# niclasborlin/dbat

Hardware: NVIDIA B200
Metric: lm_iterations_per_s (higher is better)
Workload: dtype f64

## Files before the change

dbat_b200/csrc/api.cu:

```cuda
#include <algorithm>
#include <chrono>
#include <cmath>
#include <cstdio>
#include <cstring>
#include <map>
#include <string>
#include <iterator>
#include <vector>
#include <condition_variable>
#include <functional>
#include <memory>
#include <mutex>
#include <thread>
#include <dlfcn.h>

#include "../../include/dbat_gpu.h"
#include "kernels.cuh"
#include "launch.h"
#include "tilechol.h"

int64_t g_dbat_launches = 0;
static std::string g_create_err;

#define CK(call)                                                                                   \
// ... 431 lines not shown
            for (int sl = 0; sl < DBAT_NSLOT; ++sl) {
                const int c = h->h_io_colx[(size_t)i * DBAT_NSLOT + sl];
                if (c >= 0 && lastUser[c] != i) { users[c]++; lastUser[c] = i; }
            }
        h->h_glob_x.clear();
        h->h_colLocalImg.assign(std::max(1, nC), -1);
        for (int c = 0; c < nC; ++c) {
            if (users[c] >= 2 || (users[c] == 1 && !general)) h->h_glob_x.push_back(c);
            else if (users[c] == 1) { h->h_colLocalImg[c] = lastUser[c]; h->h_nEO[lastUser[c]]++; }
        }
        h->h_nIOest = (int)h->h_glob_x.size();
        if ((rc = setup_reduced(h, 1, 0))) return fail_create(h, rc, h->err);
    }
    const std::vector<int>& imgRank = h->tc.sym.imgRank;
    AL(P.chunkG, (size_t)std::max(1, P.nChunks) * DBAT_GSZ);
    {
        const size_t nCp = (size_t)std::max(1, nC);
        h->nEvalRed = (size_t)nImg * DBAT_GSZ + DBAT_GSZ + 2 * nCp + 8;
        AL(h->d_evalRed, h->nEvalRed);
        P.imgG = h->d_evalRed;
        P.shG = P.imgG + (size_t)nImg * DBAT_GSZ;
        h->d_camDiag = P.shG + DBAT_GSZ;
        h->d_camG = h->d_camDiag + nCp;
        h->d_prr = h->d_camG + nCp;
        cudaMemset(h->d_camDiag, 0, sizeof(double) * (2 * nCp + 8));
    }
    AL(P.pt, (size_t)std::max(1, nOP) * DBAT_PT_STRIDE);
    cudaMemset(P.pt, 0, sizeof(double) * (size_t)std::max(1, nOP) * DBAT_PT_STRIDE);
    {
        bool ok = !general && nK <= 3 && nP <= 2 && getenv("DBAT_EVAL_GENERIC") == nullptr;
        for (int sl = 0; sl < DBAT_NSLOT; ++sl) if (h->h_sh_col[sl] >= 0 && !((0x0CEFu >> sl) & 1)) ok = false;
        P.evalCompact = ok ? 1 : 0;
    }
    AL(P.W, (size_t)std::max(1, nObs) * DBAT_W_STRIDE);
    if (P.ioGeneral) AL(P.Wfull, (size_t)std::max(1, nObs) * DBAT_WF_STRIDE);
    {
        std::vector<int> pt_pm(nObs);
        for (int o = 0; o < nObs; ++o) pt_pm[o] = h->h_pt_cm[h->h_pm2cm[o]];
        int* d_pt_pm;
        UP(d_pt_pm, pt_pm);
        P.pt_pm = d_pt_pm;
    }
    {
        std::vector<int> pairs, bigp;
        int begin = 0, cnt = 0;
        auto close = [&](int end) { if (end > begin) { pairs.push_back(begin); pairs.push_back(end); } begin = end; cnt = 0; };
        for (int j = 0; j < nOP; ++j) {
            const int k = h->h_pt_start[j + 1] - h->h_pt_start[j];
            if (k > DBAT_PSB) { close(j); bigp.push_back(j); begin = j + 1; continue; }
            if (cnt + k > DBAT_PSB || j - begin >= DBAT_PSB / 2) close(j);
            cnt += k;
        }
        close(nOP);
        P.nPsb = (int)pairs.size() / 2;
        P.nPsbig = (int)bigp.size();
        if (pairs.empty()) pairs.assign(2, 0);
        if (bigp.empty()) bigp.push_back(0);
        int *d_pairs, *d_bigp;
        UP(d_pairs, pairs); UP(d_bigp, bigp);
        P.psb_pt = d_pairs; P.psbig = d_bigp;
    }
    {
        std::vector<int> cand, big;
        cand.reserve(nOP);
        int maxm = DBAT_GRP_MAXM;
        if (const char* e = getenv("DBAT_GRP_MAXM")) maxm = std::max(1, std::min(DBAT_GRP_MAXM, atoi(e)));
        for (int j = 0; j < nOP; ++j) {
// ... 994 lines not shown
    res->launches = g_dbat_launches - l0;
    CK(cudaMemcpyAsync(res->x, h->d_x, sizeof(double) * nn, cudaMemcpyDeviceToHost, h->st));
    if (res->p) CK(cudaMemcpyAsync(res->p, h->d_p, sizeof(double) * nn, cudaMemcpyDeviceToHost, h->st));
    if (res->r_w || res->r_u) {
        set_params(h, h->d_x); h->params_valid = true;
        if (res->r_w) {
            launch_resid(h->P, h->d_x, h->d_partial, h->d_scal, SC_PRR, h->d_r, 1, h->st);
            CK(cudaMemcpyAsync(res->r_w, h->d_r, sizeof(double) * h->m, cudaMemcpyDeviceToHost, h->st));
            CK(cudaStreamSynchronize(h->st));
        }
        if (res->r_u) {
            launch_resid(h->P, h->d_x, h->d_partial, h->d_scal, SC_PRR, h->d_r, 0, h->st);
            CK(cudaMemcpyAsync(res->r_u, h->d_r, sizeof(double) * h->m, cudaMemcpyDeviceToHost, h->st));
        }
    }
    ph_collect(h);
    CK(cudaStreamSynchronize(h->st));
    return DBAT_OK;
}

__global__ void __launch_bounds__(128) k_cop(DevProblem P, const double* __restrict__ C, int ldc,
                                              const double* __restrict__ dsc, double s02, double* __restrict__ out);


__global__ void k_cov_rows(DevProblem P, double* __restrict__ T, int* __restrict__ Tc) {
    const int j = blockIdx.x * blockDim.x + threadIdx.x;
    if (j >= P.nOP) return;
    const size_t r0 = (size_t)DBAT_NSLOT * j + 6 * (size_t)P.pt_start[j];
    const int o0 = P.pt_start[j], k = P.pt_start[j + 1] - o0;
    const double* rec = P.pt + (size_t)j * DBAT_PT_STRIDE;
    const double* v = P.vinv + (size_t)j * 8;
    const double Vi[6] = {v[0], v[1], v[2], v[3], v[4], v[5]};
    for (int a = 0; a < DBAT_NSLOT + 6 * k; ++a) {
        const double* w; int col;
        if (a < DBAT_NSLOT) { w = rec + DBAT_PT_WSH + 3 * a; col = P.sh_s[a]; }
        else {
            const int o = (a - DBAT_NSLOT) / 6, e = (a - DBAT_NSLOT) % 6;
            w = P.W + (size_t)(o0 + o) * DBAT_W_STRIDE + 3 * e;
            col = P.eo_s[6 * (size_t)P.img_pm[o0 + o] + e];
        }
        double* t = T + 3 * (r0 + a);
        t[0] = Vi[0] * w[0] + Vi[1] * w[1] + Vi[2] * w[2];
        t[1] = Vi[1] * w[0] + Vi[3] * w[1] + Vi[4] * w[2];
        t[2] = Vi[2] * w[0] + Vi[4] * w[1] + Vi[5] * w[2];
        Tc[r0 + a] = col;
    }
}
__global__ void k_cov_U(DevProblem P, const double* __restrict__ C, int ldc, const double* __restrict__ dsc,
                        const double* __restrict__ T, const int* __restrict__ Tc, const int* __restrict__ x2s,
                        double* __restrict__ U) {
    const int rx = blockIdx.x * blockDim.x + threadIdx.x, j = blockIdx.y;
    if (rx >= P.nC) return;
    const int r = x2s[rx];
    const int* opc = P.op_col + 3 * (size_t)j;
    if (opc[0] < 0 && opc[1] < 0 && opc[2] < 0) return;
    const size_t r0 = (size_t)DBAT_NSLOT * j + 6 * (size_t)P.pt_start[j];
    const int rows = DBAT_NSLOT + 6 * (P.pt_start[j + 1] - P.pt_start[j]);
    double u[3] = {0.0, 0.0, 0.0};
    const double dr = dsc[r];
    for (int a = 0; a < rows; ++a) {
        const int ca = Tc[r0 + a];
        if (ca < 0) continue;
        const double c = C[(size_t)ca * ldc + r] * dr * dsc[ca];
        const double* t = T + 3 * (r0 + a);
        u[0] += c * t[0]; u[1] += c * t[1]; u[2] += c * t[2];
    }
    for (int t = 0; t < 3; ++t) if (opc[t] >= 0) U[(size_t)(opc[t] - P.nC) * P.nC + rx] = u[t];
}
__global__ void k_cov_pp(DevProblem P, const double* __restrict__ T, const int* __restrict__ Tc,
                         const double* __restrict__ U, const int* __restrict__ col2pt, double* __restrict__ Cpp) {
    const int m3 = P.n - P.nC;
// ... 250 lines not shown
    if (info != 0) { for (int c = 0; c < P.n; ++c) std_x[c] = NAN; return DBAT_E_NOTSPD; }
    return DBAT_OK;
}

__global__ void __launch_bounds__(128) k_cop(DevProblem P, const double* __restrict__ C, int ldc,
                                              const double* __restrict__ dsc, double s02, double* __restrict__ out) {
    const int lane = threadIdx.x & 31;
    const int j = (blockIdx.x * blockDim.x + threadIdx.x) >> 5;
    if (j >= P.nOP) return;
    const int* opc = P.op_col + 3 * (size_t)j;
    if (opc[0] < 0 && opc[1] < 0 && opc[2] < 0) return;
    const double* rec = P.pt + (size_t)j * DBAT_PT_STRIDE;
    double a00 = rec[0], a01 = rec[1], a02 = rec[2], a11 = rec[3], a12 = rec[4], a22 = rec[5];
    const bool f0 = opc[0] >= 0, f1 = opc[1] >= 0, f2 = opc[2] >= 0;
    if (!f0) a00 = 1.0; if (!f1) a11 = 1.0; if (!f2) a22 = 1.0;
    const double l00 = sqrt(a00), l10 = a01 / l00, l20 = a02 / l00;
    const double l11 = sqrt(a11 - l10 * l10), l21 = (a12 - l20 * l10) / l11;
    const double l22 = sqrt(a22 - l20 * l20 - l21 * l21);
    const double m00 = 1.0 / l00, m11 = 1.0 / l11, m22 = 1.0 / l22;
    const double m10 = -l10 * m00 * m11, m21 = -l21 * m11 * m22, m20 = -(l20 * m00 + l21 * m10) * m22;
    double Vi[6] = {m00 * m00 + m10 * m10 + m20 * m20, m10 * m11 + m20 * m21, m20 * m22,
                    m11 * m11 + m21 * m21, m21 * m22, m22 * m22};
    if (!f0) { Vi[0] = 0; Vi[1] = 0; Vi[2] = 0; }
    if (!f1) { Vi[1] = 0; Vi[3] = 0; Vi[4] = 0; }
    if (!f2) { Vi[2] = 0; Vi[4] = 0; Vi[5] = 0; }
    const int o0 = P.pt_start[j], k = P.pt_start[j + 1] - o0;
    const int nRows = DBAT_NSLOT + 6 * k;
    auto row_col = [&](int a) -> int {
        if (a < DBAT_NSLOT) return P.sh_s[a];
        const int o = (a - DBAT_NSLOT) / 6, e = (a - DBAT_NSLOT) % 6;
        return P.eo_s[6 * (size_t)P.img_pm[o0 + o] + e];
    };
    auto row_T = [&](int a, double T[3]) {
        const double* w = (a < DBAT_NSLOT) ? rec + DBAT_PT_WSH + 3 * a
                                           : P.W + (size_t)(o0 + (a - DBAT_NSLOT) / 6) * DBAT_W_STRIDE + 3 * ((a - DBAT_NSLOT) % 6);
        T[0] = Vi[0] * w[0] + Vi[1] * w[1] + Vi[2] * w[2];
        T[1] = Vi[1] * w[0] + Vi[3] * w[1] + Vi[4] * w[2];
        T[2] = Vi[2] * w[0] + Vi[4] * w[1] + Vi[5] * w[2];
    };
    double acc[6] = {0, 0, 0, 0, 0, 0};
    for (int a = lane; a < nRows; a += 32) {
        const int ca = row_col(a);
        if (ca < 0) continue;
        double Ta[3]; row_T(a, Ta);
        double u[3] = {0, 0, 0};
        for (int b = 0; b < nRows; ++b) {
            const int cb = row_col(b);
            if (cb < 0) continue;
            double Tb[3]; row_T(b, Tb);
            const double c = C[(size_t)cb * ldc + ca] * dsc[ca] * dsc[cb];
            u[0] += c * Tb[0]; u[1] += c * Tb[1]; u[2] += c * Tb[2];
        }
        acc[0] += Ta[0] * u[0]; acc[1] += Ta[0] * u[1]; acc[2] += Ta[0] * u[2];
        acc[3] += Ta[1] * u[1]; acc[4] += Ta[1] * u[2]; acc[5] += Ta[2] * u[2];
    }
#pragma unroll
    for (int q = 0; q < 6; ++q)
#pragma unroll
        for (int o = 16; o > 0; o >>= 1) acc[q] += __shfl_xor_sync(0xffffffffu, acc[q], o);
    if (lane == 0) {
        double* o9 = out + 9 * (size_t)j;
        const double c00 = s02 * (Vi[0] + acc[0]), c01 = s02 * (Vi[1] + acc[1]), c02 = s02 * (Vi[2] + acc[2]);
        const double c11 = s02 * (Vi[3] + acc[3]), c12 = s02 * (Vi[4] + acc[4]), c22 = s02 * (Vi[5] + acc[5]);
        o9[0] = c00; o9[1] = c01; o9[2] = c02; o9[3] = c01; o9[4] = c11; o9[5] = c12; o9[6] = c02; o9[7] = c12; o9[8] = c22;
    }
}

extern "C" int dbat_dense_chol_solve(int64_t n, const double* A, const double* b, double* x, double* Ainv,
// ... 452 lines not shown
```

dbat_b200/csrc/eval.cu:

```cuda
#include "kernels.cuh"
#include "launch.h"

__device__ __forceinline__ double warp_sum(double v) {
#pragma unroll
    for (int o = 16; o > 0; o >>= 1) v += __shfl_xor_sync(0xffffffffu, v, o);
    return v;
}

__device__ __forceinline__ double block_sum(double v, double* sm ) {
    v = warp_sum(v);
    const int w = threadIdx.x >> 5, l = threadIdx.x & 31;
    __syncthreads();
    if (l == 0) sm[w] = v;
    __syncthreads();
    double t = 0.0;
    if (w == 0) {
        t = (l < (int)(blockDim.x >> 5)) ? sm[l] : 0.0;
        t = warp_sum(t);
    }
    return t;
}

__global__ void __launch_bounds__(256) k_scatter3(const double* __restrict__ x, ScatterList a, ScatterList b, ScatterList c) {
    int blk = blockIdx.x;
// ... 333 lines not shown
    double m[3];
#pragma unroll
    for (int t = 0; t < 3; ++t) m[t] = P.op_col[3 * (size_t)j + t] >= 0 ? 1.0 : 0.0;
    double V[6] = {0, 0, 0, 0, 0, 0}, gq[3] = {0, 0, 0};
    double Wsh[DBAT_NSLOT][3];
#pragma unroll
    for (int s = 0; s < DBAT_NSLOT; ++s) { Wsh[s][0] = 0.0; Wsh[s][1] = 0.0; Wsh[s][2] = 0.0; }
    const int o0 = P.pt_start[j], o1 = P.pt_start[j + 1];
    for (int ob = o0; ob < o1; ++ob) {
        const double2 uv = P.uv_pm[ob];
        const double2 is = P.isig_pm[ob];
        const ImgRec g = P.img[P.img_pm[ob]];
        const IORec io = P.io[g.io];
        ObsJac o;
        obs_model<MODEL, true, true>(Q, g, io, P.nK, P.nP, uv.x, uv.y, o);
        double A[2][3];
#pragma unroll
        for (int t = 0; t < 3; ++t) { A[0][t] = o.dOP[0][t] * is.x * m[t]; A[1][t] = o.dOP[1][t] * is.y * m[t]; }
        const double r0 = o.r[0] * is.x, r1 = o.r[1] * is.y;
        V[0] += A[0][0] * A[0][0] + A[1][0] * A[1][0];
        V[1] += A[0][0] * A[0][1] + A[1][0] * A[1][1];
        V[2] += A[0][0] * A[0][2] + A[1][0] * A[1][2];
        V[3] += A[0][1] * A[0][1] + A[1][1] * A[1][1];
        V[4] += A[0][1] * A[0][2] + A[1][1] * A[1][2];
        V[5] += A[0][2] * A[0][2] + A[1][2] * A[1][2];
#pragma unroll
        for (int t = 0; t < 3; ++t) gq[t] += A[0][t] * r0 + A[1][t] * r1;
#pragma unroll
        for (int s = 0; s < DBAT_NSLOT; ++s) {
            const double a0 = o.dIO[s][0] * is.x, a1 = o.dIO[s][1] * is.y;
#pragma unroll
            for (int t = 0; t < 3; ++t) Wsh[s][t] += a0 * A[0][t] + a1 * A[1][t];
        }
        double* Wo = P.W + (size_t)ob * DBAT_W_STRIDE;
#pragma unroll
        for (int c = 0; c < 3; ++c) {
            const double a0 = o.dC[0][c] * is.x, a1 = o.dC[1][c] * is.y;
            const double b0 = o.dA[0][c] * is.x, b1 = o.dA[1][c] * is.y;
#pragma unroll
            for (int t = 0; t < 3; ++t) {
                Wo[c * 3 + t] = a0 * A[0][t] + a1 * A[1][t];
                Wo[(3 + c) * 3 + t] = b0 * A[0][t] + b1 * A[1][t];
            }
        }
    }
    double* rec = P.pt + (size_t)j * DBAT_PT_STRIDE;
#pragma unroll
    for (int k = 0; k < 6; ++k) rec[k] = V[k];
#pragma unroll
    for (int t = 0; t < 3; ++t) rec[6 + t] = gq[t];
    rec[9] = 0.0;
#pragma unroll
    for (int s = 0; s < DBAT_NSLOT; ++s)
#pragma unroll
        for (int t = 0; t < 3; ++t) rec[DBAT_PT_WSH + 3 * s + t] = Wsh[s][t];
}

__global__ void k_prior_apply(DevProblem P, const double* __restrict__ x,
                              double* __restrict__ camDiag, double* __restrict__ camG,
                              const int* __restrict__ col2pt ) {
    const int k = blockIdx.x * blockDim.x + threadIdx.x;
    if (k >= P.nPrior) return;
    const int c = P.prior_col[k];
    const double w = P.prior_isig[k];
    const double r = (x[c] - P.prior_val[k]) * w;
    if (c < P.nC) {
        camDiag[c] += w * w;
        camG[c] += w * r;
    } else {
        const int e = col2pt[c - P.nC];
        const int j = e / 3, t = e % 3;
        double* rec = P.pt + (size_t)j * DBAT_PT_STRIDE;
        const int d = (t == 0) ? 0 : (t == 1 ? 3 : 5);
        rec[d] += w * w;
        rec[6 + t] += w * r;
    }
}
// ... 7 lines not shown
    const int ob0 = P.pt_start[p0], nob = P.pt_start[p1] - ob0;
    if (tid < nob) {
        const int ob = ob0 + tid;
        const int j = P.pt_pm[ob];
        const double2 uv = P.uv_pm[ob];
        const double2 is = P.isig_pm[ob];
        const ImgRec g = P.img[P.img_pm[ob]];
        const IORec io = P.io[g.io];
        const double Q[3] = {P.OPval[3 * (size_t)j], P.OPval[3 * (size_t)j + 1], P.OPval[3 * (size_t)j + 2]};
        ObsJac o;
        obs_model<MODEL, true, true>(Q, g, io, P.nK, P.nP, uv.x, uv.y, o);
        double* row = rows + tid * PS_ROW;
        double A[2][3];
#pragma unroll
        for (int t = 0; t < 3; ++t) {
            const double m = P.op_col[3 * (size_t)j + t] >= 0 ? 1.0 : 0.0;
            A[0][t] = o.dOP[0][t] * is.x * m; A[1][t] = o.dOP[1][t] * is.y * m;
            row[t] = A[0][t]; row[3 + t] = A[1][t];
        }
        row[6] = o.r[0] * is.x; row[7] = o.r[1] * is.y;
#pragma unroll
        for (int s = 0; s < DBAT_NSLOT; ++s) { row[8 + 2 * s] = o.dIO[s][0] * is.x; row[9 + 2 * s] = o.dIO[s][1] * is.y; }
        double w[18];
#pragma unroll
        for (int c = 0; c < 3; ++c) {
            const double a0 = o.dC[0][c] * is.x, a1 = o.dC[1][c] * is.y;
            const double b0 = o.dA[0][c] * is.x, b1 = o.dA[1][c] * is.y;
#pragma unroll
            for (int t = 0; t < 3; ++t) {
                w[c * 3 + t] = a0 * A[0][t] + a1 * A[1][t];
                w[(3 + c) * 3 + t] = b0 * A[0][t] + b1 * A[1][t];
            }
        }
        double2* Wo = reinterpret_cast<double2*>(P.W + (size_t)ob * DBAT_W_STRIDE);
#pragma unroll
        for (int q = 0; q < 9; ++q) Wo[q] = make_double2(w[2 * q], w[2 * q + 1]);
    }
    __syncthreads();
    const int nItems = (p1 - p0) * 16;
    for (int item = tid; item < nItems; item += DBAT_PSB) {
        const int j = p0 + (item >> 4), it = item & 15;
        const int r0 = P.pt_start[j] - ob0, r1 = P.pt_start[j + 1] - ob0;
        double* rec = P.pt + (size_t)j * DBAT_PT_STRIDE;
        if (it < DBAT_NSLOT) {
            double a0 = 0.0, a1 = 0.0, a2 = 0.0;
            for (int r = r0; r < r1; ++r) {
                const double* row = rows + r * PS_ROW;
                const double u0 = row[8 + 2 * it], u1 = row[9 + 2 * it];
                a0 += u0 * row[0] + u1 * row[3]; a1 += u0 * row[1] + u1 * row[4]; a2 += u0 * row[2] + u1 * row[5];
            }
            rec[DBAT_PT_WSH + 3 * it] = a0; rec[DBAT_PT_WSH + 3 * it + 1] = a1; rec[DBAT_PT_WSH + 3 * it + 2] = a2;
        } else if (it == 14) {
            double V[6] = {0, 0, 0, 0, 0, 0};
            for (int r = r0; r < r1; ++r) {
                const double* row = rows + r * PS_ROW;
                V[0] += row[0] * row[0] + row[3] * row[3];
                V[1] += row[0] * row[1] + row[3] * row[4];
                V[2] += row[0] * row[2] + row[3] * row[5];
                V[3] += row[1] * row[1] + row[4] * row[4];
                V[4] += row[1] * row[2] + row[4] * row[5];
                V[5] += row[2] * row[2] + row[5] * row[5];
            }
#pragma unroll
            for (int k = 0; k < 6; ++k) rec[k] = V[k];
        } else {
            double g0 = 0.0, g1 = 0.0, g2 = 0.0;
            for (int r = r0; r < r1; ++r) {
                const double* row = rows + r * PS_ROW;
                g0 += row[0] * row[6] + row[3] * row[7]; g1 += row[1] * row[6] + row[4] * row[7]; g2 += row[2] * row[6] + row[5] * row[7];
            }
            rec[6] = g0; rec[7] = g1; rec[8] = g2; rec[9] = 0.0;
        }
    }
}

#define PSC_ROW 27
__device__ __constant__ unsigned char c_ceSlot[CE_NA] = {0, 1, 2, 3, 5, 6, 7, 10, 11};
#ifndef PSC_MINB
#define PSC_MINB 5
#endif
template <int MODEL>
__global__ void __launch_bounds__(DBAT_PSB, PSC_MINB) k_point_side_obs_c(DevProblem P) {
    __shared__ __align__(16) double rows[DBAT_PSB * PSC_ROW];
    const int tid = threadIdx.x, lane = tid & 31;
    const int p0 = P.psb_pt[2 * blockIdx.x], p1 = P.psb_pt[2 * blockIdx.x + 1];
    const int ob0 = P.pt_start[p0], nob = P.pt_start[p1] - ob0;
    const bool valid = tid < nob;
    ObsJac o;
    double A[2][3];
    double2 is = make_double2(0.0, 0.0);
    double* stage = rows + (tid - lane) * PSC_ROW;
    if (valid) {
        const int ob = ob0 + tid;
        const int j = P.pt_pm[ob];
        const double2 uv = P.uv_pm[ob];
        is = P.isig_pm[ob];
        const ImgRec g = P.img[P.img_pm[ob]];
        const IORec io = P.io[g.io];
        const double Q[3] = {P.OPval[3 * (size_t)j], P.OPval[3 * (size_t)j + 1], P.OPval[3 * (size_t)j + 2]};
        obs_model<MODEL, true, true>(Q, g, io, CE_NK, CE_NP, uv.x, uv.y, o);
#pragma unroll
        for (int t = 0; t < 3; ++t) {
            const double m = P.op_col[3 * (size_t)j + t] >= 0 ? 1.0 : 0.0;
            A[0][t] = o.dOP[0][t] * is.x * m; A[1][t] = o.dOP[1][t] * is.y * m;
        }
        double w[18];
#pragma unroll
        for (int c = 0; c < 3; ++c) {
            const double a0 = o.dC[0][c] * is.x, a1 = o.dC[1][c] * is.y;
            const double b0 = o.dA[0][c] * is.x, b1 = o.dA[1][c] * is.y;
#pragma unroll
            for (int t = 0; t < 3; ++t) {
                w[c * 3 + t] = a0 * A[0][t] + a1 * A[1][t];
                w[(3 + c) * 3 + t] = b0 * A[0][t] + b1 * A[1][t];
            }
        }
        double2* sw = reinterpret_cast<double2*>(stage + lane * DBAT_W_STRIDE);
#pragma unroll
        for (int q = 0; q < 9; ++q) sw[q] = make_double2(w[2 * q], w[2 * q + 1]);
    }
    __syncwarp();
    {
        const int nv = min(32, nob - (tid - lane));
        double2* Wg = reinterpret_cast<double2*>(P.W + (size_t)(ob0 + tid - lane) * DBAT_W_STRIDE);
        const double2* ss = reinterpret_cast<const double2*>(stage);
#pragma unroll
        for (int q = 0; q < 9; ++q) {
            const int piece = q * 32 + lane;
            if (piece < nv * 9) Wg[piece] = ss[piece];
        }
    }
    __syncwarp();
    if (valid) {
        double* row = rows + tid * PSC_ROW;
#pragma unroll
        for (int t = 0; t < 3; ++t) { row[t] = A[0][t]; row[3 + t] = A[1][t]; }
        row[6] = o.r[0] * is.x; row[7] = o.r[1] * is.y;
#pragma unroll
        for (int s = 0; s < DBAT_NSLOT; ++s) {
            if ((CE_MASK >> s) & 1) { row[8 + ce_col(s)] = o.dIO[s][0] * is.x; row[8 + CE_NA + ce_col(s)] = o.dIO[s][1] * is.y; }
        }
    }
    __syncthreads();
    {
        const int warp = tid >> 5;
        const int fm = lane >> 2, fk = lane & 3;
        const int xy = fk & 1, oo = fk >> 1;
        const int nB = 8 + fm;
        const int offA = 3 * xy + fm;
        const int offB0 = fm < 3 ? 3 * xy + fm : (fm == 3 ? 6 + xy : 8 + CE_NA * xy + (fm - 4));
        const bool b1ok = nB < 4 + CE_NA;
        const int offB1 = 8 + CE_NA * xy + (nB - 4);
        for (int jj = warp; jj < p1 - p0; jj += DBAT_PSB / 32) {
            const int j = p0 + jj;
            const int r0 = P.pt_start[j] - ob0, r1 = P.pt_start[j + 1] - ob0;
            double c00 = 0.0, c01 = 0.0, c10 = 0.0, c11 = 0.0;
            for (int r = r0; r < r1; r += 2) {
                const int ro = r + oo;
                const bool in = ro < r1;
                const double* row = rows + ro * PSC_ROW;
                const double a = (in && fm < 3) ? row[offA] : 0.0;
                const double b0 = in ? row[offB0] : 0.0;
                const double b1 = (in && b1ok) ? row[offB1] : 0.0;
                dmma884(c00, c01, a, b0);
                dmma884(c10, c11, a, b1);
            }
// ... 296 lines not shown
```

dbat_b200/csrc/kernels.cuh:

```cuda
#pragma once
#include <cstdint>
#include <cuda_runtime.h>
#include "model.cuh"
#include "tilechol.h"

#define DBAT_GW 24
#define DBAT_GT 3
#define DBAT_GTP 6
#define DBAT_GSZ (DBAT_GTP * 64)
#define DBAT_COL_EO DBAT_NSLOT
#define DBAT_COL_R (DBAT_NSLOT + 6)
#define DBAT_PSB 128
#define DBAT_CHUNK 1024
#define DBAT_PT_STRIDE 52
#define DBAT_PT_WSH 10
#define DBAT_W_STRIDE 18
#define DBAT_NCAM (DBAT_NSLOT + 6)
#define DBAT_WF_STRIDE (3 * DBAT_NCAM)

static_assert(DBAT_NSLOT + 7 <= DBAT_GW, "Gram width");

struct Chunk { int img, start, count, pad; };

#define WIN_GP 14
#define WIN_MAXW 20
struct __align__(16) WinHdr {
    int m, ng, p0, pad;
    int j[WIN_GP];
    int ob[WIN_GP];
    unsigned char wslot[WIN_MAXW];
    unsigned char obsOf[WIN_GP][WIN_MAXW];
    unsigned char pad2[4];
};
static_assert(sizeof(WinHdr) == 432, "WinHdr layout");

struct DevProblem {
    int nImg, nOP, nObs, nK, nP, model;
    int n;
    int nC;
    int nChunks;
    int ldS;
    int nPrior;
    const double2* uv_cm; const double2* isig_cm; const int* pt_cm; const int* img_cm;
    const double2* uv_pm; const double2* isig_pm; const int* img_pm; const int* pm2cm;
    const int* pt_start;
    const int* psb_pt;
    int nPsb;
    const int* psbig;
    int nPsbig;
// ... 16 lines not shown
    const int* glob_x;
    TCholDev T;
    const int* prior_col; const double* prior_val; const double* prior_isig;
    double* chunkG;
    double* imgG;
    double* shG;
    double* pt;
    double* W;
    double* rhs;
    const int* pt_pm;
    const int* grp_pt;
    int grpMaxRays;
    const int* big_pt;
    int nBig;
    double* vinv;
    const WinHdr* win_hdr;
    const int* clu_grp;
    const int* clu_order;
    const int* clu_img_off;
    const int* clu_img;
    const long long* clu_stg;
    int nClu, nCand;
    double* winM;
    double* win_stg;
    const int* red_ptr;
    const int* red_imgA; const int* red_imgB;
    const long long* red_off;
    int nRedBlk;
    const int* redi_ptr;
    const long long* redi_off;
    double* win_ssPart;
};
#define DBAT_GRP_MAXM 20
```

dbat_b200/csrc/schur.cu:

```cuda
#include "kernels.cuh"
#include <algorithm>
#include "launch.h"

__device__ __forceinline__ double gram_at(const double* __restrict__ G, int R, int C) {
    if (R < C) { const int t = R; R = C; C = t; }
    const int p = R >> 3, q = C >> 3, i = R & 7, j = C & 7;
    const int tp = p * (p + 1) / 2 + q;
    return G[tp * 64 + (i * 4 + (j >> 1)) * 2 + (j & 1)];
}

__device__ __forceinline__ bool point_inverse(const double* __restrict__ rec, const int* __restrict__ opc,
                                              double lambda, double Vi[6]) {
    double a00 = rec[0], a01 = rec[1], a02 = rec[2], a11 = rec[3], a12 = rec[4], a22 = rec[5];
    const bool f0 = opc[0] >= 0, f1 = opc[1] >= 0, f2 = opc[2] >= 0;
    a00 = f0 ? a00 + lambda : 1.0;
    a11 = f1 ? a11 + lambda : 1.0;
    a22 = f2 ? a22 + lambda : 1.0;
    bool ok = a00 > 0.0;
    const double l00 = sqrt(a00);
    const double l10 = a01 / l00, l20 = a02 / l00;
    const double d1 = a11 - l10 * l10;
    ok = ok && d1 > 0.0;
    const double l11 = sqrt(d1);
    const double l21 = (a12 - l20 * l10) / l11;
// ... 107 lines not shown
}

__global__ void __launch_bounds__(256) k_schur_atomic(DevProblem P, double lambda, double* __restrict__ shAcc,
                                                      const int* __restrict__ list, int nList) {
    const int lane = threadIdx.x & 31;
    const int warpGlobal = (blockIdx.x * blockDim.x + threadIdx.x) >> 5;
    const int nWarps = (gridDim.x * blockDim.x) >> 5;
    constexpr int NE = DBAT_NSLOT * (DBAT_NSLOT + 1);
    constexpr int NEL = (NE + 31) / 32;
    double accSh[NEL];
#pragma unroll
    for (int k = 0; k < NEL; ++k) accSh[k] = 0.0;

    for (int jj = warpGlobal; jj < nList; jj += nWarps) {
        const int j = list[jj];
        const double* rec = P.pt + (size_t)j * DBAT_PT_STRIDE;
        const int* opc = P.op_col + 3 * (size_t)j;
        if (opc[0] < 0 && opc[1] < 0 && opc[2] < 0) continue;
        double Vi[6];
        point_inverse(rec, opc, lambda, Vi);
        const double gj[3] = {rec[6], rec[7], rec[8]};
        double Vg[3];
        symv3(Vi, gj, Vg);
        const int o0 = P.pt_start[j], k = P.pt_start[j + 1] - o0;
        const int nItems = k * (k + 1) / 2 * 6;
        for (int it = lane; it < nItems; it += 32) {
            const int pr = it / 6, a = it - pr * 6;
            int o = (int)((sqrt(8.0 * pr + 1.0) - 1.0) * 0.5);
            while ((o + 1) * (o + 2) / 2 <= pr) ++o;
            while (o * (o + 1) / 2 > pr) --o;
            const int o2 = pr - o * (o + 1) / 2;
            const int row = P.eo_s[6 * (size_t)P.img_pm[o0 + o] + a];
            if (row < 0) continue;
            const double* Wa = P.W + (size_t)(o0 + o) * DBAT_W_STRIDE + 3 * a;
            const double wa[3] = {Wa[0], Wa[1], Wa[2]};
            double ya[3];
            symv3(Vi, wa, ya);
            const int* ec2 = P.eo_s + 6 * (size_t)P.img_pm[o0 + o2];
            const double* Wb = P.W + (size_t)(o0 + o2) * DBAT_W_STRIDE;
#pragma unroll
            for (int b = 0; b < 6; ++b) {
                const int col = ec2[b];
                if (col < 0 || (o2 == o && col > row)) continue;
                const double v = ya[0] * Wb[3 * b] + ya[1] * Wb[3 * b + 1] + ya[2] * Wb[3 * b + 2];
                atomicAdd(tc_at(P.T, max(row, col), min(row, col)), -v);
            }
            if (o2 == 0) {
                atomicAdd(&P.rhs[row], ya[0] * gj[0] + ya[1] * gj[1] + ya[2] * gj[2]);
#pragma unroll
                for (int s = 0; s < DBAT_NSLOT; ++s) {
                    const int srow = P.sh_s[s];
                    if (srow < 0) continue;
                    const double* ws = rec + DBAT_PT_WSH + 3 * s;
                    atomicAdd(tc_at(P.T, srow, row), -(ya[0] * ws[0] + ya[1] * ws[1] + ya[2] * ws[2]));
                }
            }
        }
#pragma unroll
        for (int kk = 0; kk < NEL; ++kk) {
            const int e = lane + 32 * kk;
            if (e < NE) {
                const int a = e / (DBAT_NSLOT + 1), b = e - a * (DBAT_NSLOT + 1);
                const double* wa = rec + DBAT_PT_WSH + 3 * a;
                if (b < DBAT_NSLOT) {
                    if (b <= a) {
                        const double* wb = rec + DBAT_PT_WSH + 3 * b;
                        const double w3[3] = {wb[0], wb[1], wb[2]};
                        double y[3];
                        symv3(Vi, w3, y);
                        accSh[kk] += wa[0] * y[0] + wa[1] * y[1] + wa[2] * y[2];
                    }
                } else {
                    accSh[kk] += wa[0] * Vg[0] + wa[1] * Vg[1] + wa[2] * Vg[2];
                }
            }
        }
    }
// ... 60 lines not shown
    pEO[t] = v;
}
void launch_unpermute(const DevProblem& P, const double* xs, const double* d, double* pc, double* pEO, cudaStream_t st) {
    const int nbS = (P.ldS + 255) / 256, nbE = pEO ? (6 * P.nImg + 255) / 256 : 0;
    k_unpermute<<<nbS + nbE, 256, 0, st>>>(P, xs, d, pc, pEO, nbS);
    count_launch();
}

__global__ void __launch_bounds__(128) k_backsub(DevProblem P, double lambda, double* __restrict__ p,
                                                  double* __restrict__ stats, int statStride,
                                                  const int* __restrict__ list, int nList) {
    __shared__ double red[2][4];
    const int jj = blockIdx.x * blockDim.x + threadIdx.x;
    const int j = jj < nList ? list[jj] : P.nOP;
    double jp2 = 0.0, rjp = 0.0;
    if (j < P.nOP) {
        const int* opc = P.op_col + 3 * (size_t)j;
        if (!(opc[0] < 0 && opc[1] < 0 && opc[2] < 0)) {
            const double* rec = P.pt + (size_t)j * DBAT_PT_STRIDE;
            double Vi[6];
            point_inverse(rec, opc, lambda, Vi);
            double a[3] = {0.0, 0.0, 0.0};
#pragma unroll
            for (int s = 0; s < DBAT_NSLOT; ++s) {
                const int c = P.sh_col[s];
                if (c < 0) continue;
                const double pv = p[c];
                const double* ws = rec + DBAT_PT_WSH + 3 * s;
                a[0] += ws[0] * pv; a[1] += ws[1] * pv; a[2] += ws[2] * pv;
            }
            const int o0 = P.pt_start[j], o1 = P.pt_start[j + 1];
            for (int ob = o0; ob < o1; ++ob) {
                const int* ec = P.eo_col + 6 * (size_t)P.img_pm[ob];
                const double* Wo = P.W + (size_t)ob * DBAT_W_STRIDE;
#pragma unroll
                for (int e = 0; e < 6; ++e) {
                    const int c = ec[e];
                    if (c < 0) continue;
                    const double pv = p[c];
                    a[0] += Wo[3 * e] * pv; a[1] += Wo[3 * e + 1] * pv; a[2] += Wo[3 * e + 2] * pv;
                }
            }
            const double t[3] = {-rec[6] - a[0], -rec[7] - a[1], -rec[8] - a[2]};
            double y[3];
            symv3(Vi, t, y);
#pragma unroll
            for (int e = 0; e < 3; ++e) if (opc[e] >= 0) p[opc[e]] = y[e]; else y[e] = 0.0;
            const double Vy0 = rec[0] * y[0] + rec[1] * y[1] + rec[2] * y[2];
            const double Vy1 = rec[1] * y[0] + rec[3] * y[1] + rec[4] * y[2];
            const double Vy2 = rec[2] * y[0] + rec[4] * y[1] + rec[5] * y[2];
            jp2 = y[0] * (Vy0 + 2.0 * a[0]) + y[1] * (Vy1 + 2.0 * a[1]) + y[2] * (Vy2 + 2.0 * a[2]);
            rjp = rec[6] * y[0] + rec[7] * y[1] + rec[8] * y[2];
        }
    }
    if (stats) {
#pragma unroll
        for (int o = 16; o > 0; o >>= 1) { jp2 += __shfl_xor_sync(0xffffffffu, jp2, o); rjp += __shfl_xor_sync(0xffffffffu, rjp, o); }
        if ((threadIdx.x & 31) == 0) { red[0][threadIdx.x >> 5] = jp2; red[1][threadIdx.x >> 5] = rjp; }
        __syncthreads();
        if (threadIdx.x == 0) {
            stats[blockIdx.x] = (red[0][0] + red[0][1]) + (red[0][2] + red[0][3]);
            stats[statStride + blockIdx.x] = (red[1][0] + red[1][1]) + (red[1][2] + red[1][3]);
        }
    }
}
__global__ void __launch_bounds__(DBAT_PSB) k_backsub_obs(DevProblem P, double lambda, double* __restrict__ p,
                                                           const double* __restrict__ pEO,
                                                           double* __restrict__ stats, int statStride) {
    __shared__ double ao[DBAT_PSB * 3];
    __shared__ double red[2][DBAT_PSB / 32];
    __shared__ double psh[DBAT_NSLOT + 2];
    __shared__ int pshOk[DBAT_NSLOT + 2];
    const int tid = threadIdx.x;
    const int p0 = P.psb_pt[2 * blockIdx.x], p1 = P.psb_pt[2 * blockIdx.x + 1];
    const int ob0 = P.pt_start[p0], nob = P.pt_start[p1] - ob0;
    if (p0 + tid < p1) {
        const char* rec = reinterpret_cast<const char*>(P.pt + (size_t)(p0 + tid) * DBAT_PT_STRIDE);
#pragma unroll
        for (int b = 0; b < DBAT_PT_STRIDE * 8; b += 128) asm volatile("prefetch.global.L1 [%0];" :: "l"(rec + b));
        asm volatile("prefetch.global.L1 [%0];" :: "l"(rec + DBAT_PT_STRIDE * 8 - 8));
        asm volatile("prefetch.global.L1 [%0];" :: "l"(P.op_col + 3 * (size_t)(p0 + tid)));
    }
    if (tid >= DBAT_PSB - DBAT_NSLOT) {
        const int s = tid - (DBAT_PSB - DBAT_NSLOT);
        const int c = P.sh_col[s];
        psh[s] = c >= 0 ? p[c] : 0.0;
        pshOk[s] = c >= 0;
    }
    if (tid < nob) {
        const int ob = ob0 + tid;
        const double2* Wo = reinterpret_cast<const double2*>(P.W + (size_t)ob * DBAT_W_STRIDE);
        double w[18];
#pragma unroll
        for (int q = 0; q < 9; ++q) { const double2 t = Wo[q]; w[2 * q] = t.x; w[2 * q + 1] = t.y; }
        double a0 = 0.0, a1 = 0.0, a2 = 0.0;
        const double2* pe = reinterpret_cast<const double2*>(pEO + 6 * (size_t)P.img_pm[ob]);
        const double2 e01 = pe[0], e23 = pe[1], e45 = pe[2];
        const double pv[6] = {e01.x, e01.y, e23.x, e23.y, e45.x, e45.y};
#pragma unroll
        for (int e = 0; e < 6; ++e) { a0 += w[3 * e] * pv[e]; a1 += w[3 * e + 1] * pv[e]; a2 += w[3 * e + 2] * pv[e]; }
        ao[3 * tid] = a0; ao[3 * tid + 1] = a1; ao[3 * tid + 2] = a2;
    }
    __syncthreads();
    double jp2 = 0.0, rjp = 0.0;
    const int j = p0 + tid;
    if (j < p1) {
        const int* opc = P.op_col + 3 * (size_t)j;
        if (!(opc[0] < 0 && opc[1] < 0 && opc[2] < 0)) {
            const double* rec = P.pt + (size_t)j * DBAT_PT_STRIDE;
            double Vi[6];
            point_inverse(rec, opc, lambda, Vi);
            double a[3] = {0.0, 0.0, 0.0};
#pragma unroll
            for (int s = 0; s < DBAT_NSLOT; ++s) {
                if (!pshOk[s]) continue;
                const double pv = psh[s];
                const double* ws = rec + DBAT_PT_WSH + 3 * s;
                a[0] += ws[0] * pv; a[1] += ws[1] * pv; a[2] += ws[2] * pv;
            }
            for (int r = P.pt_start[j] - ob0; r < P.pt_start[j + 1] - ob0; ++r) { a[0] += ao[3 * r]; a[1] += ao[3 * r + 1]; a[2] += ao[3 * r + 2]; }
            const double t[3] = {-rec[6] - a[0], -rec[7] - a[1], -rec[8] - a[2]};
            double y[3];
            symv3(Vi, t, y);
#pragma unroll
            for (int e = 0; e < 3; ++e) if (opc[e] >= 0) p[opc[e]] = y[e]; else y[e] = 0.0;
            const double Vy0 = rec[0] * y[0] + rec[1] * y[1] + rec[2] * y[2];
            const double Vy1 = rec[1] * y[0] + rec[3] * y[1] + rec[4] * y[2];
            const double Vy2 = rec[2] * y[0] + rec[4] * y[1] + rec[5] * y[2];
            jp2 = y[0] * (Vy0 + 2.0 * a[0]) + y[1] * (Vy1 + 2.0 * a[1]) + y[2] * (Vy2 + 2.0 * a[2]);
            rjp = rec[6] * y[0] + rec[7] * y[1] + rec[8] * y[2];
        }
    }
    if (stats) {
#pragma unroll
        for (int o = 16; o > 0; o >>= 1) { jp2 += __shfl_xor_sync(0xffffffffu, jp2, o); rjp += __shfl_xor_sync(0xffffffffu, rjp, o); }
        if ((tid & 31) == 0) { red[0][tid >> 5] = jp2; red[1][tid >> 5] = rjp; }
        __syncthreads();
        if (tid == 0) {
            double s0 = 0.0, s1 = 0.0;
#pragma unroll
            for (int w = 0; w < DBAT_PSB / 32; ++w) { s0 += red[0][w]; s1 += red[1][w]; }
            stats[blockIdx.x] = s0; stats[statStride + blockIdx.x] = s1;
        }
    }
}
__global__ void __launch_bounds__(128) k_jp_cam(DevProblem P, const double* __restrict__ p,
                                                 const double* __restrict__ camDiag, const double* __restrict__ camG,
                                                 double* __restrict__ stats) {
    __shared__ double red[2][4];
    __shared__ double vs[4][DBAT_NSLOT + 6 + 2];
    const int lane = threadIdx.x & 31, warp = threadIdx.x >> 5;
// ... 157 lines not shown
```

dbat_b200/csrc/schur_win.cu:

```cuda
#include <algorithm>
#include <cstdio>
#include <vector>
#include "kernels.cuh"
#include "launch.h"

#ifndef WIN_TH
#define WIN_TH 256
#endif
#ifndef WIN_UNIT
#define WIN_UNIT 3
#endif
#define WIN_SHLD (6 * WIN_MAXW)
#define WIN_NBLK (WIN_MAXW * (WIN_MAXW + 1) / 2)
#define WIN_ACC (WIN_NBLK * 36)
#define WIN_MAXRT ((6 * WIN_MAXW + 7) / 8)
#define WIN_MAXUNIT 96
#define WIN_SSPART 256

__constant__ unsigned int c_winUnits[WIN_MAXRT + 1][WIN_MAXUNIT];
__constant__ int c_winNUnits[WIN_MAXRT + 1];

static void build_units(unsigned int (*tab)[WIN_MAXUNIT], int* cnt) {
    for (int RT = 0; RT <= WIN_MAXRT; ++RT) {
        std::vector<unsigned int> u;
// ... 57 lines not shown
        }
    }
#pragma unroll
    for (int n = 0; n < CNT; ++n) { c[n][0] += d[n][0]; c[n][1] += d[n][1]; }
}

template <int LDR>
__global__ void __launch_bounds__(WIN_TH, 2) k_schur_win(DevProblem P) {
    extern __shared__ __align__(16) double dsm[];
    __shared__ __align__(16) WinHdr s_hdr[3];
    __shared__ __align__(16) double s_M[2][WIN_GP * 6];
    __shared__ int s_rowTab[8 * WIN_MAXRT], s_colTab[4 * WIN_MAXRT], s_colSh[4 * WIN_MAXRT];
    const int t = threadIdx.x, lane = t & 31, warp = t >> 5;
    const int fr = lane >> 2, fk = lane & 3;
    const int RTmaxP = (6 * P.grpMaxRays + 7) >> 3;
    const int shRow0 = 8 * RTmaxP;
    constexpr int ZT = (3 * WIN_GP + 2) * LDR;
    double* Zt = dsm;
    double* Acc = Zt + ZT;
    double* AccSh = Acc + WIN_ACC;
    double* AccSS = AccSh + 16 * WIN_SHLD;
    const int clu = P.clu_order[blockIdx.x];
    const int g0 = P.clu_grp[clu], g1 = P.clu_grp[clu + 1];
    const int mw = P.clu_img_off[clu + 1] - P.clu_img_off[clu];
    for (int i = t; i < (ZT + WIN_ACC + 16 * WIN_SHLD + 256) / 2; i += WIN_TH)
        reinterpret_cast<double2*>(dsm)[i] = make_double2(0.0, 0.0);
    auto cell_load = [&](const WinHdr& H, int idx, int mq, unsigned inv, double2 (&w)[9]) {
        const int gi = (int)(((unsigned)idx * inv) >> 24), q = idx - gi * mq;
#pragma unroll
        for (int k = 0; k < 9; ++k) w[k] = make_double2(0.0, 0.0);
        if (q < mq - 3) {
            const int o = H.obsOf[gi][q];
            if (o != 255) {
                const double2* p = reinterpret_cast<const double2*>(P.W + (size_t)(H.ob[gi] + o) * DBAT_W_STRIDE);
#pragma unroll
                for (int k = 0; k < 9; ++k) w[k] = p[k];
            }
        } else {
            const int b = q - (mq - 3);
            const double2* rec = reinterpret_cast<const double2*>(P.pt + (size_t)H.j[gi] * DBAT_PT_STRIDE);
            if (b < 2) {
#pragma unroll
                for (int k = 0; k < 9; ++k) w[k] = rec[5 + 9 * b + k];
            } else {
                w[0] = rec[23]; w[1] = rec[24]; w[2] = rec[25];
                const double2 g01 = rec[3], g2 = rec[4];
                w[3] = g01; w[4] = make_double2(g2.x, 0.0);
            }
        }
    };
    auto cell_put = [&](const WinHdr& H, const double* Ms, int idx, int mq, unsigned inv, const double2 (&w)[9]) {
        const int gi = (int)(((unsigned)idx * inv) >> 24), q = idx - gi * mq;
        const int row0 = q < mq - 3 ? 6 * q : shRow0 + 6 * (q - (mq - 3));
        const double* Mg = Ms + 6 * gi;
        const double m00 = Mg[0], m10 = Mg[1], m11 = Mg[2], m20 = Mg[3], m21 = Mg[4], m22 = Mg[5];
        double* z = Zt + (3 * gi) * LDR + row0;
        const double* wd = reinterpret_cast<const double*>(w);
#pragma unroll
        for (int a = 0; a < 6; ++a) {
            const double w0 = wd[3 * a], w1 = wd[3 * a + 1], w2 = wd[3 * a + 2];
            z[a] = w0 * m00;
            z[LDR + a] = w0 * m10 + w1 * m11;
            z[2 * LDR + a] = w0 * m20 + w1 * m21 + w2 * m22;
        }
    };
    double2 cw[9];
    auto load_cells = [&](const WinHdr& H) {
        const int mq = H.m + 3;
        const unsigned inv = (0x1000000u + mq - 1) / mq;
// ... 238 lines not shown
```

Baseline: 528.9.

## Interleave W rows in blocks of four observations for coalesced double2 access

Changes the per-observation W buffer from row-major stride-18 to a blocked layout where pairs of doubles from four consecutive observations sit next to each other. Every producer and consumer (eval, schur, schur_win, covariance kernels) now goes through w_load/w_store2 helpers, so adjacent threads touch contiguous 16-byte pairs. This removes the warp-level shared-memory staging in one eval kernel. It also vectorises the shared-slot W reads in the back-substitution into double2 loads. Scalar readers such as the Schur atomics and covariance kernels now pay extra index arithmetic and may lose contiguity.

```diff
diff --git a/dbat_b200/csrc/api.cu b/dbat_b200/csrc/api.cu
--- a/dbat_b200/csrc/api.cu
+++ b/dbat_b200/csrc/api.cu
@@ -487,7 +487,7 @@
         for (int sl = 0; sl < DBAT_NSLOT; ++sl) if (h->h_sh_col[sl] >= 0 && !((0x0CEFu >> sl) & 1)) ok = false;
         P.evalCompact = ok ? 1 : 0;
     }
-    AL(P.W, (size_t)std::max(1, nObs) * DBAT_W_STRIDE);
+    AL(P.W, w_doubles(std::max(1, nObs)));
     if (P.ioGeneral) AL(P.Wfull, (size_t)std::max(1, nObs) * DBAT_WF_STRIDE);
     {
         std::vector<int> pt_pm(nObs);
@@ -1548,11 +1548,15 @@
     const double* v = P.vinv + (size_t)j * 8;
     const double Vi[6] = {v[0], v[1], v[2], v[3], v[4], v[5]};
     for (int a = 0; a < DBAT_NSLOT + 6 * k; ++a) {
-        const double* w; int col;
-        if (a < DBAT_NSLOT) { w = rec + DBAT_PT_WSH + 3 * a; col = P.sh_s[a]; }
-        else {
+        double w[3]; int col;
+        if (a < DBAT_NSLOT) {
+            const double* ws = rec + DBAT_PT_WSH + 3 * a;
+            w[0] = ws[0]; w[1] = ws[1]; w[2] = ws[2];
+            col = P.sh_s[a];
+        } else {
             const int o = (a - DBAT_NSLOT) / 6, e = (a - DBAT_NSLOT) % 6;
-            w = P.W + (size_t)(o0 + o) * DBAT_W_STRIDE + 3 * e;
+#pragma unroll
+            for (int t = 0; t < 3; ++t) w[t] = w_load(P.W, o0 + o, 3 * e + t);
             col = P.eo_s[6 * (size_t)P.img_pm[o0 + o] + e];
         }
         double* t = T + 3 * (r0 + a);
@@ -1869,8 +1873,15 @@
         return P.eo_s[6 * (size_t)P.img_pm[o0 + o] + e];
     };
     auto row_T = [&](int a, double T[3]) {
-        const double* w = (a < DBAT_NSLOT) ? rec + DBAT_PT_WSH + 3 * a
-                                           : P.W + (size_t)(o0 + (a - DBAT_NSLOT) / 6) * DBAT_W_STRIDE + 3 * ((a - DBAT_NSLOT) % 6);
+        double w[3];
+        if (a < DBAT_NSLOT) {
+            const double* ws = rec + DBAT_PT_WSH + 3 * a;
+            w[0] = ws[0]; w[1] = ws[1]; w[2] = ws[2];
+        } else {
+            const int o = (a - DBAT_NSLOT) / 6, e = (a - DBAT_NSLOT) % 6;
+#pragma unroll
+            for (int t = 0; t < 3; ++t) w[t] = w_load(P.W, o0 + o, 3 * e + t);
+        }
         T[0] = Vi[0] * w[0] + Vi[1] * w[1] + Vi[2] * w[2];
         T[1] = Vi[1] * w[0] + Vi[3] * w[1] + Vi[4] * w[2];
         T[2] = Vi[2] * w[0] + Vi[4] * w[1] + Vi[5] * w[2];
diff --git a/dbat_b200/csrc/eval.cu b/dbat_b200/csrc/eval.cu
--- a/dbat_b200/csrc/eval.cu
+++ b/dbat_b200/csrc/eval.cu
@@ -389,17 +389,19 @@
 #pragma unroll
             for (int t = 0; t < 3; ++t) Wsh[s][t] += a0 * A[0][t] + a1 * A[1][t];
         }
-        double* Wo = P.W + (size_t)ob * DBAT_W_STRIDE;
+        double w[18];
 #pragma unroll
         for (int c = 0; c < 3; ++c) {
             const double a0 = o.dC[0][c] * is.x, a1 = o.dC[1][c] * is.y;
             const double b0 = o.dA[0][c] * is.x, b1 = o.dA[1][c] * is.y;
 #pragma unroll
             for (int t = 0; t < 3; ++t) {
-                Wo[c * 3 + t] = a0 * A[0][t] + a1 * A[1][t];
-                Wo[(3 + c) * 3 + t] = b0 * A[0][t] + b1 * A[1][t];
+                w[c * 3 + t] = a0 * A[0][t] + a1 * A[1][t];
+                w[(3 + c) * 3 + t] = b0 * A[0][t] + b1 * A[1][t];
             }
         }
+#pragma unroll
+        for (int q = 0; q < 9; ++q) w_store2(P.W, ob, q, make_double2(w[2 * q], w[2 * q + 1]));
     }
     double* rec = P.pt + (size_t)j * DBAT_PT_STRIDE;
 #pragma unroll
@@ -473,9 +475,8 @@
                 w[(3 + c) * 3 + t] = b0 * A[0][t] + b1 * A[1][t];
             }
         }
-        double2* Wo = reinterpret_cast<double2*>(P.W + (size_t)ob * DBAT_W_STRIDE);
-#pragma unroll
-        for (int q = 0; q < 9; ++q) Wo[q] = make_double2(w[2 * q], w[2 * q + 1]);
+#pragma unroll
+        for (int q = 0; q < 9; ++q) w_store2(P.W, ob, q, make_double2(w[2 * q], w[2 * q + 1]));
     }
     __syncthreads();
     const int nItems = (p1 - p0) * 16;
@@ -526,20 +527,17 @@
     const int tid = threadIdx.x, lane = tid & 31;
     const int p0 = P.psb_pt[2 * blockIdx.x], p1 = P.psb_pt[2 * blockIdx.x + 1];
     const int ob0 = P.pt_start[p0], nob = P.pt_start[p1] - ob0;
-    const bool valid = tid < nob;
-    ObsJac o;
-    double A[2][3];
-    double2 is = make_double2(0.0, 0.0);
-    double* stage = rows + (tid - lane) * PSC_ROW;
-    if (valid) {
+    if (tid < nob) {
         const int ob = ob0 + tid;
         const int j = P.pt_pm[ob];
         const double2 uv = P.uv_pm[ob];
-        is = P.isig_pm[ob];
+        const double2 is = P.isig_pm[ob];
         const ImgRec g = P.img[P.img_pm[ob]];
         const IORec io = P.io[g.io];
         const double Q[3] = {P.OPval[3 * (size_t)j], P.OPval[3 * (size_t)j + 1], P.OPval[3 * (size_t)j + 2]};
+        ObsJac o;
         obs_model<MODEL, true, true>(Q, g, io, CE_NK, CE_NP, uv.x, uv.y, o);
+        double A[2][3];
 #pragma unroll
         for (int t = 0; t < 3; ++t) {
             const double m = P.op_col[3 * (size_t)j + t] >= 0 ? 1.0 : 0.0;
@@ -556,23 +554,8 @@
                 w[(3 + c) * 3 + t] = b0 * A[0][t] + b1 * A[1][t];
             }
         }
-        double2* sw = reinterpret_cast<double2*>(stage + lane * DBAT_W_STRIDE);
-#pragma unroll
-        for (int q = 0; q < 9; ++q) sw[q] = make_double2(w[2 * q], w[2 * q + 1]);
-    }
-    __syncwarp();
-    {
-        const int nv = min(32, nob - (tid - lane));
-        double2* Wg = reinterpret_cast<double2*>(P.W + (size_t)(ob0 + tid - lane) * DBAT_W_STRIDE);
-        const double2* ss = reinterpret_cast<const double2*>(stage);
-#pragma unroll
-        for (int q = 0; q < 9; ++q) {
-            const int piece = q * 32 + lane;
-            if (piece < nv * 9) Wg[piece] = ss[piece];
-        }
-    }
-    __syncwarp();
-    if (valid) {
+#pragma unroll
+        for (int q = 0; q < 9; ++q) w_store2(P.W, ob, q, make_double2(w[2 * q], w[2 * q + 1]));
         double* row = rows + tid * PSC_ROW;
 #pragma unroll
         for (int t = 0; t < 3; ++t) { row[t] = A[0][t]; row[3 + t] = A[1][t]; }
diff --git a/dbat_b200/csrc/kernels.cuh b/dbat_b200/csrc/kernels.cuh
--- a/dbat_b200/csrc/kernels.cuh
+++ b/dbat_b200/csrc/kernels.cuh
@@ -15,6 +15,7 @@
 #define DBAT_PT_STRIDE 52
 #define DBAT_PT_WSH 10
 #define DBAT_W_STRIDE 18
+#define DBAT_W_BLK 4
 #define DBAT_NCAM (DBAT_NSLOT + 6)
 #define DBAT_WF_STRIDE (3 * DBAT_NCAM)
 
@@ -97,3 +98,20 @@
     double* win_ssPart;
 };
 #define DBAT_GRP_MAXM 20
+
+inline size_t w_doubles(int nObs) {
+    return (size_t)((nObs + DBAT_W_BLK - 1) / DBAT_W_BLK) * DBAT_W_BLK * DBAT_W_STRIDE;
+}
+__device__ __forceinline__ size_t w_pair(int o, int q) {
+    const unsigned u = (unsigned)o;
+    return (size_t)(u / DBAT_W_BLK) * (DBAT_W_BLK * DBAT_W_STRIDE / 2) + q * DBAT_W_BLK + (u % DBAT_W_BLK);
+}
+__device__ __forceinline__ double2 w_load2(const double* W, int o, int q) {
+    return reinterpret_cast<const double2*>(W)[w_pair(o, q)];
+}
+__device__ __forceinline__ void w_store2(double* W, int o, int q, double2 v) {
+    reinterpret_cast<double2*>(W)[w_pair(o, q)] = v;
+}
+__device__ __forceinline__ double w_load(const double* W, int o, int k) {
+    return W[2 * w_pair(o, k >> 1) + (k & 1)];
+}
diff --git a/dbat_b200/csrc/schur.cu b/dbat_b200/csrc/schur.cu
--- a/dbat_b200/csrc/schur.cu
+++ b/dbat_b200/csrc/schur.cu
@@ -163,17 +163,16 @@
             const int o2 = pr - o * (o + 1) / 2;
             const int row = P.eo_s[6 * (size_t)P.img_pm[o0 + o] + a];
             if (row < 0) continue;
-            const double* Wa = P.W + (size_t)(o0 + o) * DBAT_W_STRIDE + 3 * a;
-            const double wa[3] = {Wa[0], Wa[1], Wa[2]};
+            const double wa[3] = {w_load(P.W, o0 + o, 3 * a), w_load(P.W, o0 + o, 3 * a + 1), w_load(P.W, o0 + o, 3 * a + 2)};
             double ya[3];
             symv3(Vi, wa, ya);
             const int* ec2 = P.eo_s + 6 * (size_t)P.img_pm[o0 + o2];
-            const double* Wb = P.W + (size_t)(o0 + o2) * DBAT_W_STRIDE;
 #pragma unroll
             for (int b = 0; b < 6; ++b) {
                 const int col = ec2[b];
                 if (col < 0 || (o2 == o && col > row)) continue;
-                const double v = ya[0] * Wb[3 * b] + ya[1] * Wb[3 * b + 1] + ya[2] * Wb[3 * b + 2];
+                const double v = ya[0] * w_load(P.W, o0 + o2, 3 * b) + ya[1] * w_load(P.W, o0 + o2, 3 * b + 1)
+                               + ya[2] * w_load(P.W, o0 + o2, 3 * b + 2);
                 atomicAdd(tc_at(P.T, max(row, col), min(row, col)), -v);
             }
             if (o2 == 0) {
@@ -300,13 +299,12 @@
             const int o0 = P.pt_start[j], o1 = P.pt_start[j + 1];
             for (int ob = o0; ob < o1; ++ob) {
                 const int* ec = P.eo_col + 6 * (size_t)P.img_pm[ob];
-                const double* Wo = P.W + (size_t)ob * DBAT_W_STRIDE;
 #pragma unroll
                 for (int e = 0; e < 6; ++e) {
                     const int c = ec[e];
                     if (c < 0) continue;
                     const double pv = p[c];
-                    a[0] += Wo[3 * e] * pv; a[1] += Wo[3 * e + 1] * pv; a[2] += Wo[3 * e + 2] * pv;
+                    a[0] += w_load(P.W, ob, 3 * e) * pv; a[1] += w_load(P.W, ob, 3 * e + 1) * pv; a[2] += w_load(P.W, ob, 3 * e + 2) * pv;
                 }
             }
             const double t[3] = {-rec[6] - a[0], -rec[7] - a[1], -rec[8] - a[2]};
@@ -357,10 +355,9 @@
     }
     if (tid < nob) {
         const int ob = ob0 + tid;
-        const double2* Wo = reinterpret_cast<const double2*>(P.W + (size_t)ob * DBAT_W_STRIDE);
         double w[18];
 #pragma unroll
-        for (int q = 0; q < 9; ++q) { const double2 t = Wo[q]; w[2 * q] = t.x; w[2 * q + 1] = t.y; }
+        for (int q = 0; q < 9; ++q) { const double2 t = w_load2(P.W, ob, q); w[2 * q] = t.x; w[2 * q + 1] = t.y; }
         double a0 = 0.0, a1 = 0.0, a2 = 0.0;
         const double2* pe = reinterpret_cast<const double2*>(pEO + 6 * (size_t)P.img_pm[ob]);
         const double2 e01 = pe[0], e23 = pe[1], e45 = pe[2];
@@ -379,12 +376,14 @@
             double Vi[6];
             point_inverse(rec, opc, lambda, Vi);
             double a[3] = {0.0, 0.0, 0.0};
-#pragma unroll
-            for (int s = 0; s < DBAT_NSLOT; ++s) {
-                if (!pshOk[s]) continue;
-                const double pv = psh[s];
-                const double* ws = rec + DBAT_PT_WSH + 3 * s;
-                a[0] += ws[0] * pv; a[1] += ws[1] * pv; a[2] += ws[2] * pv;
+            static_assert(DBAT_PT_STRIDE % 2 == 0 && DBAT_PT_WSH % 2 == 0 && DBAT_NSLOT % 2 == 0, "IO rows of the point record in 16-byte pairs");
+            const double2* ws = reinterpret_cast<const double2*>(rec + DBAT_PT_WSH);
+#pragma unroll
+            for (int s = 0; s < DBAT_NSLOT; s += 2) {
+                if (!pshOk[s] && !pshOk[s + 1]) continue;
+                const double2 w0 = ws[3 * (s / 2)], w1 = ws[3 * (s / 2) + 1], w2 = ws[3 * (s / 2) + 2];
+                if (pshOk[s]) { const double pv = psh[s]; a[0] += w0.x * pv; a[1] += w0.y * pv; a[2] += w1.x * pv; }
+                if (pshOk[s + 1]) { const double pv = psh[s + 1]; a[0] += w1.y * pv; a[1] += w2.x * pv; a[2] += w2.y * pv; }
             }
             for (int r = P.pt_start[j] - ob0; r < P.pt_start[j + 1] - ob0; ++r) { a[0] += ao[3 * r]; a[1] += ao[3 * r + 1]; a[2] += ao[3 * r + 2]; }
             const double t[3] = {-rec[6] - a[0], -rec[7] - a[1], -rec[8] - a[2]};
diff --git a/dbat_b200/csrc/schur_win.cu b/dbat_b200/csrc/schur_win.cu
--- a/dbat_b200/csrc/schur_win.cu
+++ b/dbat_b200/csrc/schur_win.cu
@@ -113,9 +113,8 @@
         if (q < mq - 3) {
             const int o = H.obsOf[gi][q];
             if (o != 255) {
-                const double2* p = reinterpret_cast<const double2*>(P.W + (size_t)(H.ob[gi] + o) * DBAT_W_STRIDE);
-#pragma unroll
-                for (int k = 0; k < 9; ++k) w[k] = p[k];
+#pragma unroll
+                for (int k = 0; k < 9; ++k) w[k] = w_load2(P.W, H.ob[gi] + o, k);
             }
         } else {
             const int b = q - (mq - 3);
```

After: 535.6 (median of 6 runs). +1.3%, better.
